# liangheming/simple_pose

Hardware: AMD Instinct MI355X
Metric: images/sec fwd+decode, ResNet50-DConv 256x192 bs=128 (higher is better)
Workload: dtype f32; 1 GPU; ResNet50-DConv 256x192 bs=128 per GPU, fp32 forward (NCHW in -> heat maps) + GaussTaylor decode, eval-mode BN, conditioned random weights; images_per_gpu=128, global_batch=128, parallelism=replicas x1 (no collective), ranks=1 process(es), one per GPU, launch=stream launches, tile_table=profiles/r06_dconv_f32_tiles.json, batches_in_flight=2, decode=in line, HSA_ENABLE_IPC_MODE_LEGACY=0

## Files before the change

### include/simple_pose_hip.h

```cpp
#ifndef SIMPLE_POSE_HIP_H
#define SIMPLE_POSE_HIP_H

#include <stdint.h>

#ifdef __cplusplus
extern "C" {
#endif

#define SP_OK 0
#define SP_EINVAL (-1)
#define SP_ELAUNCH (-2)

#define SP_ABI_VERSION 36

#define SP_CONV_RELU 0x1u
#define SP_CONV_OUT_NCHW 0x2u
#define SP_CONV_PIXEL_SHUFFLE 0x4u
#define SP_CONV_OUT_F32 0x10u
#define SP_CONV_BN_Y_MASK 0x20u
#define SP_CONV_BF16 0x8u
#define SP_CONV_HARDSWISH 0x40u
#define SP_CONV_OUT_SLICE 0x80u

typedef struct sp_conv_desc {
// ... 26 lines not shown


int sp_nchw_to_nhwc4(const float* x_nchw, float* y_nhwc4, int batch, int channels, int h, int w, void* stream);

int sp_conv2d_fwd(const sp_conv_desc* desc, const void* x, const void* w_packed, const float* scale,
                  const float* shift, const void* residual, void* y, void* stream);

int sp_conv_set_tap_skip(int on);

int sp_conv3x3_direct_ok(const sp_conv_desc* desc);
int sp_conv3x3_direct(const sp_conv_desc* desc, const void* x, const void* w_packed, const float* scale, const float* shift,
                      const void* residual, void* y, void* stream);

int sp_basic_block_c32_ok(const sp_conv_desc* desc);
int sp_basic_block_c32(const sp_conv_desc* desc, const void* x, const void* w1_packed, const float* scale1, const float* shift1,
                       const void* w2_packed, const float* scale2, const float* shift2, void* y, void* stream);

int sp_basic_block_c64_ok(const sp_conv_desc* desc);
int sp_basic_block_c64(const sp_conv_desc* desc, const void* x, const void* w1_packed, const float* scale1, const float* shift1,
                       const void* w2_packed, const float* scale2, const float* shift2, void* y, void* stream);

int sp_dual_pw_bf16_ok(int64_t rows, int c_main, int c_short, int c_out);
int sp_dual_pw_f32_ok(int64_t rows, int c_main, int c_short, int c_out);
int sp_dual_pw_f32(const float* a_main, const float* w_main_packed, const float* scale_main, const float* shift_main, const float* a_short,
                   const float* w_short_packed, const float* scale_short, const float* shift_short, float* y, int64_t rows, int c_main, int c_short,
                   int c_out, int relu, void* stream);
int sp_dual_pw_bf16(const void* a_main, const void* w_main_packed, const float* scale_main, const float* shift_main, const void* a_short,
                    const void* w_short_packed, const float* scale_short, const float* shift_short, void* y, int64_t rows, int c_main, int c_short,
                    int c_out, int relu, void* stream);
int sp_pw_chain_f32_ok(int64_t rows, int c_mid, int c_out, int c_next);
int sp_pw_chain_f32(const float* t, const float* w3_packed, const float* scale3, const float* shift3, const float* residual, float* y,
                    const float* w1_packed, const float* scale1, const float* shift1, float* t_next, int64_t rows, int c_mid, int c_out, int c_next,
                    void* stream);
int sp_bottleneck_c64_ok(const sp_conv_desc* desc);
int sp_bottleneck_c64(const sp_conv_desc* desc, const void* x, const void* w1_packed, const float* scale1, const float* shift1,
                      const void* w2_packed, const float* scale2, const float* shift2, const void* w3_packed, const float* scale3,
                      const float* shift3, void* y, void* stream);

int sp_stem7_pool_ok(int batch, int h, int w);
int sp_stem7_pool(const float* x, const void* w_packed, int k_pad, const float* scale, const float* shift, void* y, int bf16,
                  int batch, int h, int w, void* stream);
int sp_stem7_pool_u8(const unsigned char* crops_bgr, const float* mean_rgb_host, const void* w_packed, int k_pad, const float* scale,
                     const float* shift, void* y, int bf16, int batch, int h, int w, void* stream);

int sp_hrnet_transition1_ok(int c_in, int h, int w);
int sp_hrnet_transition1(const void* x, int batch, int h, int w, const void* wa_packed, int k_pad, const float* scale_a, const float* shift_a,
                         const void* wb_packed, const float* scale_b, const float* shift_b, void* y_hi, void* y_lo, void* stream);
int sp_hrnet_stem_ok(int batch, int h, int w);
int sp_hrnet_stem(const float* x, const void* w1_packed, int k1_pad, const float* scale1, const float* shift1, const void* w2_packed,
                  const float* scale2, const float* shift2, void* y, int batch, int h, int w, void* stream);

int sp_conv2d_pw_ok(const sp_conv_desc* desc);

int sp_conv2d_ring_ok(const sp_conv_desc* desc);

int sp_conv2d_kernel_name(const sp_conv_desc* desc, int has_residual, int variant, char* buf, int cap);

int sp_conv2d_default_tile(const sp_conv_desc* desc, int* tile_m, int* tile_n);

int sp_maxpool3x3s2_nhwc(const float* x, float* y, int batch, int h, int w, int c, void* stream);

int sp_pixel_shuffle2_nhwc(const float* x, float* y, int batch, int h, int w, int c, void* stream);

int sp_global_avg_pool_nhwc(const float* x, float* y, int batch, int hw, int c, void* stream);
int sp_se_gate_add_relu_nhwc(const float* x, const float* gate_logits, const float* identity, float* y, int batch, int hw,
                             int c, void* stream);
// ... 360 lines not shown
```

### simple_pose_amd/_lib.py

```python
from __future__ import annotations

import ctypes
import os
from ctypes import c_double, c_float, c_int, c_int32, c_int64, c_uint32, c_void_p

from .build import LIB_PATH as _DEFAULT_LIB_PATH

LIB_PATH = os.environ.get("SIMPLE_POSE_HIP_LIB", _DEFAULT_LIB_PATH)

SP_CONV_RELU = 0x1
SP_CONV_OUT_NCHW = 0x2
SP_CONV_PIXEL_SHUFFLE = 0x4
SP_CONV_BF16 = 0x8
SP_CONV_OUT_F32 = 0x10
SP_CONV_BN_Y_MASK = 0x20
SP_CONV_HARDSWISH = 0x40
SP_CONV_OUT_SLICE = 0x80
SP_LETTERBOX_FOCUS, SP_LETTERBOX_U8 = 0, 1
SP_YOLO_NMS_MAX_CANDIDATES, SP_YOLO_NMS_MAX_DET = 32768, 1024
SP_COCO_MAX_JOINTS, SP_COCO_MAX_GT_PER_IMAGE, SP_COCO_MAX_DT_PER_IMAGE, SP_COCO_MAX_DETS = 64, 128, 2048, 32
SP_COCO_DT_XY_F64, SP_COCO_DT_SCORE_F64, SP_COCO_GT_CROWD, SP_COCO_GT_IGNORE = 1, 2, 1, 2
CONV_TILES =((128, 128), (64, 128), (128, 64), (64, 64), (256, 64), (128, 32))
ABI_VERSION = 36
SP_CONV_KERNEL_IGEMM, SP_CONV_KERNEL_RING, SP_CONV_KERNEL_PW, SP_CONV_KERNEL_RING_LW, SP_CONV_KERNEL_RING_LW4 = 0, 1, 2, 3, 4
# ... 138 lines not shown
    "sp_pixel_unshuffle2_nhwc_bf16": (c_int, [_P, _P, c_int, c_int, c_int, c_int, _P]),
    "sp_maxpool3x3s2_idx_nhwc": (c_int, [_P, c_int, _P, _P, c_int, c_int, c_int, c_int, _P]),
    "sp_maxpool3x3s2_bwd_idx_nhwc": (c_int, [_P, _P, c_int, _P, c_int, c_int, c_int, c_int, _P]),
    "sp_nchw_to_nhwc_pad": (c_int, [_P, _P, c_int, c_int, c_int, c_int, c_int, c_int, _P]),
    "sp_warp_affine_u8c3": (c_int, [_P, c_int, c_int, _P, c_int, _P, c_int, c_int, _P]),
    "sp_warp_affine_batch_u8c3_to_nchw_f32": (c_int, [_P, _P, _P, _P, c_int, c_int, c_int, ctypes.POINTER(c_float), _P, _P, _P]),
    "sp_conv2d_bn_stats_rows": (c_int, [ctypes.POINTER(ConvDesc), ctypes.POINTER(c_int)]),
    "sp_conv2d_fwd_bn_stats": (c_int, [ctypes.POINTER(ConvDesc), _P, _P, _P, _P, _P, c_int, _P]),
    "sp_conv2d_fwd_bn_stats_abn": (c_int, [ctypes.POINTER(ConvDesc), _P, _P, _P, _P, _P, _P, _P, _P, _P, _P, _P, c_int, _P]),
    "sp_bn_train_stats_from_conv": (c_int, [_P, _P, c_int, c_int, c_int64, c_int, c_float, c_float, _P, _P, _P, _P, _P]),
    "sp_conv2d_dgrad_bn_bwd_stats": (c_int, [ctypes.POINTER(ConvDesc), _P, _P, _P, _P, _P, _P, _P, _P, _P, _P, c_int, _P]),
    "sp_conv2d_dgrad_bn_bwd_stats2": (c_int, [ctypes.POINTER(ConvDesc), _P, _P, _P, _P, _P, _P, _P, _P, _P, _P, _P, _P, _P, _P, c_int, _P]),
    "sp_conv2d_dgrad_bn_bwd_stats_macc": (c_int, [ctypes.POINTER(ConvDesc), _P, _P, _P, _P, _P, _P, _P, _P, _P, _P, _P, _P, _P, _P, _P, c_int, _P]),
    "sp_conv2d_dgrad_phases": (c_int, [ctypes.POINTER(ConvDesc), c_int, _P, ctypes.POINTER(_P), _P, _P, _P, _P, _P, _P, _P, _P, _P, _P, _P, _P, c_int, _P]),
    "sp_bn_sums_from_conv": (c_int, [_P, _P, c_int, c_int, c_int, _P, _P]),
    "sp_bn_fold_apply_nhwc": (c_int, [_P, c_int, _P, _P, c_int, c_int, c_int64, c_float, c_float, _P, _P, _P, _P, c_int64, c_int, c_int, _P, _P, _P, _P, _P, _P]),
    "sp_bn_fold_bwd_apply_nhwc": (c_int, [_P, c_int, _P, _P, _P, _P, _P, c_int, c_int, _P, _P, _P, c_int64, c_int64, c_int, _P, _P, _P, _P, _P, _P, c_int, _P]),
    "sp_bn_bwd_sums_from_conv": (c_int, [_P, _P, c_int, c_int, c_int, _P, _P, _P]),
    "sp_bn_bwd_sums_from_conv_pair": (c_int, [_P, _P, _P, c_int, c_int, c_int, _P, _P, _P, _P, _P]),
    "sp_u8hwc_bgr_to_nhwc": (c_int, [_P, _P, c_int, c_int, c_int, c_int, _P, _P]),
    "sp_nchw_to_nhwc4_bf16": (c_int, [_P, _P, c_int, c_int, c_int, c_int, _P]),
    "sp_conv3x3_direct_ok": (c_int, [ctypes.POINTER(ConvDesc)]),
    "sp_conv3x3_direct": (c_int, [ctypes.POINTER(ConvDesc), _P, _P, _P, _P, _P, _P, _P]),
    "sp_basic_block_c32_ok": (c_int, [ctypes.POINTER(ConvDesc)]),
    "sp_basic_block_c32": (c_int, [ctypes.POINTER(ConvDesc), _P, _P, _P, _P, _P, _P, _P, _P, _P]),
    "sp_basic_block_c64_ok": (c_int, [ctypes.POINTER(ConvDesc)]),
    "sp_basic_block_c64": (c_int, [ctypes.POINTER(ConvDesc), _P, _P, _P, _P, _P, _P, _P, _P, _P]),
    "sp_dual_pw_bf16_ok": (c_int, [c_int64, c_int, c_int, c_int]),
    "sp_dual_pw_f32_ok": (c_int, [c_int64, c_int, c_int, c_int]),
    "sp_dual_pw_f32": (c_int, [_P, _P, _P, _P, _P, _P, _P, _P, _P, c_int64, c_int, c_int, c_int, c_int, _P]),
    "sp_dual_pw_bf16": (c_int, [_P, _P, _P, _P, _P, _P, _P, _P, _P, c_int64, c_int, c_int, c_int, c_int, _P]),
    "sp_pw_chain_f32_ok": (c_int, [c_int64, c_int, c_int, c_int]),
    "sp_pw_chain_f32": (c_int, [_P, _P, _P, _P, _P, _P, _P, _P, _P, _P, c_int64, c_int, c_int, c_int, _P]),
    "sp_bottleneck_c64_ok": (c_int, [ctypes.POINTER(ConvDesc)]),
    "sp_conv2d_pw_ok": (c_int, [ctypes.POINTER(ConvDesc)]),
    "sp_hrnet_stem_ok": (c_int, [c_int, c_int, c_int]),
    "sp_hrnet_stem": (c_int, [_P, _P, c_int, _P, _P, _P, _P, _P, _P, c_int, c_int, c_int, _P]),
    "sp_hrnet_transition1_ok": (c_int, [c_int, c_int, c_int]),
    "sp_hrnet_transition1": (c_int, [_P, c_int, c_int, c_int, _P, c_int, _P, _P, _P, _P, _P, _P, _P, _P]),
    "sp_stem7_pool_ok": (c_int, [c_int, c_int, c_int]),
    "sp_stem7_pool": (c_int, [_P, _P, c_int, _P, _P, _P, c_int, c_int, c_int, c_int, _P]),
    "sp_stem7_pool_u8": (c_int, [_P, ctypes.POINTER(ctypes.c_float), _P, c_int, _P, _P, _P, c_int, c_int, c_int, c_int, _P]),
    "sp_bottleneck_c64": (c_int, [ctypes.POINTER(ConvDesc), _P, _P, _P, _P, _P, _P, _P, _P, _P, _P, _P, _P]),
    "sp_masked_mse": (c_int, [_P, _P, _P, c_int, c_int, c_int, _P, _P, _P, _P]),
    "sp_conv_packed_dims": (c_int, [c_int, c_int, c_int, ctypes.POINTER(c_int), ctypes.POINTER(c_int)]),
    "sp_pack_conv_weights": (c_int, [_P, c_int, c_int, c_int, c_int, c_int, c_int, c_int, c_int, c_int, c_int, _P, c_int, _P]),
    "sp_pack_conv_weights_grouped": (c_int, [_P, c_int, c_int, c_int, c_int, c_int, _P, c_int, _P]),
    "sp_pack_conv_weights_grouped_taps": (c_int, [_P, c_int, c_int, c_int, c_int, c_int, c_int, c_int, c_int, c_int, c_int, c_int, c_int, _P, c_int, _P]),
    "sp_conv2d_wgrad_grouped_workspace": (c_int, [c_int, c_int, c_int, c_int, c_int, c_int, ctypes.POINTER(c_int64)]),
    "sp_conv2d_wgrad_grouped": (c_int, [_P, _P, c_int, c_int, c_int, c_int, c_int, c_int, c_int, c_int, c_int, c_int, c_int, c_int, _P, _P, c_int64, _P]),
    "sp_pack_deconv_k4s2p1": (c_int, [_P, c_int, c_int, c_int, _P, c_int, _P]),
    "sp_fold_bn": (c_int, [_P, _P, _P, _P, c_int, c_float, c_int, _P, _P, _P]),
    "sp_yolo_letterbox": (c_int, [_P, c_int, c_int, c_int, c_int, c_int, c_int, c_int, c_int, c_int, c_int, _P, _P]),
    "sp_yolo_focus_nchw": (c_int, [_P, c_int, c_int, c_int, _P, _P]),
    "sp_yolo_spp_nhwc": (c_int, [_P, c_int, c_int, c_int, c_int, c_int, _P]),
    "sp_upsample2_slice_nhwc": (c_int, [_P, c_int, _P, c_int, c_int, c_int, c_int, c_int, _P]),
    "sp_yolo_head_decode": (c_int, [_P, _P, _P, c_int, ctypes.POINTER(c_int32), c_int, c_int, c_int, ctypes.POINTER(c_float), ctypes.POINTER(c_float), _P, _P]),
    "sp_yolo_nms_workspace": (c_int, [c_int, ctypes.POINTER(c_int64)]),
    "sp_yolo_nms": (c_int, [_P, c_int, c_int, c_int, c_float, c_float, c_int, c_int, c_int, c_int, _P, c_int64, _P, ctypes.POINTER(c_int32), ctypes.POINTER(c_int32), _P]),
    "sp_yolo_boxes_to_source": (c_int, [_P, c_int, c_float, c_float, c_float, c_float, c_float, _P]),
    "sp_yolo_nms_device": (c_int, [_P, c_int, c_int, c_int, c_float, c_float, c_int, c_int, c_int, c_int, _P, c_int64, _P, _P, _P, _P]),
    "sp_topdown_plan": (c_int, [_P, _P, c_int, c_int, c_int, c_float, c_int, c_int, c_int, c_int, c_int, _P, _P, _P, _P, _P, _P, _P, _P, _P, _P, _P]),
    "sp_warp_affine_plan_u8c3": (c_int, [_P, c_int, c_int, c_int, _P, _P, _P, c_int, _P, c_int, c_int, _P]),
    "sp_mirror_w": (c_int, [_P, _P, c_int64, c_int, c_int, _P]),
    "sp_heat_map_flip_merge": (c_int, [_P, _P, ctypes.POINTER(c_int32), c_int, c_int, c_int, c_int, c_int, _P, _P]),
    "sp_track_associate": (c_int, [_P, _P, _P, _P, _P, _P, c_int, c_int, ctypes.POINTER(c_double), c_double, c_int, c_int, _P, _P, _P, _P, _P, _P, _P, _P,
# ... 104 lines not shown
```

### simple_pose_amd/csrc/conv_pw.hip

```cpp
#include "sp_common.h"

namespace {

struct PwArgs {
    const float* x;
    const float* w;
    const float* scale;
    const float* shift;
    const float* res;
    float* y;
    int M, N, nchunks, tiles_m, relu;
    unsigned x_bytes, y_bytes;
};

constexpr int BM = 64;
constexpr int TRS = 68;
constexpr unsigned OOB = 0x80000000u;

template <int K>
__global__ __launch_bounds__(256, 1) void conv_pw_kernel(const PwArgs p) {
    constexpr int CH = K / 4;
    constexpr int NG = K / 8;
    constexpr int APT = BM * CH / 256;
    extern __shared__ __align__(16) float smem[];
// ... 403 lines not shown
#pragma unroll
        for (int i = 0; i < RT; ++i) fy[0][i] = yfrag(i, 0);
#pragma unroll
        for (int g = 0; g < NG1; ++g) {
            if (g + 1 < NG1) {
#pragma unroll
                for (int i = 0; i < RT; ++i) fy[(g + 1) & 1][i] = yfrag(i, g + 1);
            }
#pragma unroll
            for (int s = 0; s < 4; ++s)
#pragma unroll
                for (int i = 0; i < RT; ++i) c[i] = __builtin_amdgcn_mfma_f32_32x32x2f32(fy[g & 1][i][s], fw[g][s], c[i], 0, 0, 0);
        }
#pragma unroll
        for (int i = 0; i < RT; ++i)
#pragma unroll
            for (int r = 0; r < 16; ++r) {
                float v = c[i][r] * s1v + h1v;
                v = v > 0.f ? v : 0.f;
                t2[(i * 32 + (r & 3) + 8 * (r >> 2) + 4 * fh) * T2S + fr] = v;
            }
#pragma unroll
        for (int it = 0; it < RT * 4; ++it) {
            const int lr = it * 8 + (lane >> 3), cc = (lane & 7) * 4;
            const int row = m0 + ri0 * 32 + lr;
            const unsigned o = row < p.M ? (unsigned)(((size_t)row * NEXT + cn * 32 + cc) * 4) : OOB;
            const f32x4 v = *reinterpret_cast<const f32x4*>(t2 + lr * T2S + cc);
            __builtin_amdgcn_raw_buffer_store_b128(__builtin_bit_cast(u32x4, v), tnr, o, 0, 0);
        }
        __syncthreads();
    }
}

template <int NEXT>
int launch_pw_chain(const PwChainArgs& a, hipStream_t stream) {
    constexpr int lds = (2 * BM * 64 + 4 * BM * TRS + 4 * (NEXT / 64) * 32 * T2S) * 4;
    if (sp_reserve_lds<&conv_pw_chain_kernel<64, NEXT>>(lds, "conv_pw_chain")) return SP_ELAUNCH;
    int slots = sp_device_cus();
    if (slots < 1) slots = 1;
    if (slots > a.tiles_m) slots = a.tiles_m;
    const int rounds = (a.tiles_m + slots - 1) / slots;
    slots = (a.tiles_m + rounds - 1) / rounds;
    hipLaunchKernelGGL((conv_pw_chain_kernel<64, NEXT>), dim3(slots), dim3(256), lds, stream, a);
    return sp_check_launch("conv_pw_chain_kernel");
}

template <int K>
int launch_pw_dual(const PwDualArgs& a, hipStream_t stream) {
    constexpr int lds = (4 * BM * K + 4 * BM * TRS) * 4;
    if (sp_reserve_lds<&conv_pw_dual_kernel<K>>(lds, "conv_pw_dual")) return SP_ELAUNCH;
    int slots = sp_device_cus() / a.nchunks;
    if (slots < 1) slots = 1;
    if (slots > a.tiles_m) slots = a.tiles_m;
    const int rounds = (a.tiles_m + slots - 1) / slots;
    slots = (a.tiles_m + rounds - 1) / rounds;
    hipLaunchKernelGGL(conv_pw_dual_kernel<K>, dim3(slots * a.nchunks), dim3(256), lds, stream, a);
    return sp_check_launch("conv_pw_dual_kernel");
}

template <int K>
int launch_pw(const PwArgs& a, hipStream_t stream) {
    constexpr int lds = (2 * BM * K + 4 * BM * TRS) * 4;
    if (sp_reserve_lds<&conv_pw_kernel<K>>(lds, "conv_pw")) return SP_ELAUNCH;
    int slots = sp_device_cus() / a.nchunks;
    if (slots < 1) slots = 1;
    if (slots > a.tiles_m) slots = a.tiles_m;
// ... 46 lines not shown
    SP_REQUIRE(a_main && w_main_packed && a_short && w_short_packed && y, "sp_dual_pw_f32: null pointer");
    SP_REQUIRE(sp_dual_pw_f32_ok(rows, c_main, c_short, c_out), "sp_dual_pw_f32: two fp32 1x1 stride-1 products of 64 channels each into a multiple of 256 (got %d + %d -> %d, %lld rows)",
               c_main, c_short, c_out, (long long)rows);
    SP_REQUIRE(y != a_main && y != a_short, "sp_dual_pw_f32: y must not alias an input");
    if (sp_name_query_active()) { sp_name_query_set("conv_pw_dual_kernel<64>"); return SP_OK; }
    PwDualArgs a;
    a.x_main = a_main; a.x_short = a_short; a.w_main = w_main_packed; a.w_short = w_short_packed;
    a.s_main = scale_main; a.h_main = shift_main; a.s_short = scale_short; a.h_short = shift_short; a.y = y;
    a.M = (int)rows; a.N = c_out; a.nchunks = c_out / 256; a.tiles_m = (int)((rows + BM - 1) / BM); a.relu = relu ? 1 : 0;
    a.x_bytes = (unsigned)(rows * 64 * 4); a.y_bytes = (unsigned)(rows * c_out * 4);
    return launch_pw_dual<64>(a, (hipStream_t)stream);
}

extern "C" int sp_pw_chain_f32_ok(int64_t rows, int c_mid, int c_out, int c_next) {
    return rows > 0 && rows * (int64_t)c_out <= (1ll << 29) && c_mid == 64 && c_out == 256 && (c_next == 64 || c_next == 128);
}

extern "C" int sp_pw_chain_f32(const float* t, const float* w3_packed, const float* scale3, const float* shift3, const float* residual, float* y,
                               const float* w1_packed, const float* scale1, const float* shift1, float* t_next, int64_t rows, int c_mid, int c_out,
                               int c_next, void* stream) {
    SP_REQUIRE(t && w3_packed && residual && y && w1_packed && t_next, "sp_pw_chain_f32: null pointer");
    SP_REQUIRE(sp_pw_chain_f32_ok(rows, c_mid, c_out, c_next),
               "sp_pw_chain_f32: an fp32 1x1 product 64 -> 256 chained into a 1x1 product 256 -> 64 or 128 (got %d -> %d -> %d, %lld rows)", c_mid, c_out,
               c_next, (long long)rows);
    SP_REQUIRE(y != t && y != residual && t_next != t && t_next != residual && t_next != y, "sp_pw_chain_f32: y and t_next must not alias an input or each other");
    if (sp_name_query_active()) { sp_name_query_set("conv_pw_chain_kernel<64, %d>", c_next); return SP_OK; }
    PwChainArgs a;
    a.x = t; a.w = w3_packed; a.scale = scale3; a.shift = shift3; a.res = residual; a.y = y;
    a.w1 = w1_packed; a.scale1 = scale1; a.shift1 = shift1; a.t = t_next;
    a.M = (int)rows; a.tiles_m = (int)((rows + BM - 1) / BM);
    a.x_bytes = (unsigned)(rows * 64 * 4); a.y_bytes = (unsigned)(rows * 256 * 4); a.t_bytes = (unsigned)(rows * c_next * 4);
    return c_next == 64 ? launch_pw_chain<64>(a, (hipStream_t)stream) : launch_pw_chain<128>(a, (hipStream_t)stream);
}
```

### simple_pose_amd/engine.py

```python
from __future__ import annotations

import ctypes
import os

from dataclasses import dataclass, field
from typing import Dict, List, Optional, Tuple

import torch

from . import _lib, conv_geometry
from ._lib import ConvDesc, SP_CONV_BF16, SP_CONV_HARDSWISH, SP_CONV_OUT_NCHW, SP_CONV_OUT_SLICE, SP_CONV_PIXEL_SHUFFLE, SP_CONV_RELU
from .conv_geometry import n_pad_for, round_up as _round_up

BN_EPS = 1e-5


class HipPacker:

    @staticmethod
    def _dims(c_out: int, k: int, bf16: bool) -> Tuple[int, int]:
        n_pad, k_pad = ctypes.c_int(0), ctypes.c_int(0)
        _lib.check(_lib.lib().sp_conv_packed_dims(c_out, k, int(bf16), ctypes.byref(n_pad), ctypes.byref(k_pad)), "sp_conv_packed_dims")
        return n_pad.value, k_pad.value

# ... 147 lines not shown
                last_writer[dn] = i
            for n in op.reads() + op.writes():
                touched.setdefault(store(n), []).append(i)
        records = sorted({j for w in waits for j in w})
        tails: Dict[int, int] = {}
        for i, op in enumerate(self.ops):
            tails[op.lane] = i
        self._sync[key] = (waits, set(records), tails)
        return self._sync[key]

    def _lane_streams(self, key, n_lanes: int, device=None) -> list:
        pool = self._streams.setdefault(str(key), [])
        while len(pool) < n_lanes - 1:
            pool.append(torch.cuda.Stream(device=device if device is not None else key))
        return pool

    def _launch(self, lib, op: Op, bufs, B: int, stream) -> None:
        P = _lib.ptr
        if op.kind == "conv":
            op.desc.batch = B
            fn = lib.sp_conv3x3_direct if op.direct else lib.sp_conv2d_fwd
            _lib.check(fn(op.desc, P(bufs[op.src]), P(op.w), P(op.scale), P(op.shift),
                          P(bufs[op.res]) if op.res else None, P(bufs[op.dst]) + 4 * op.c0, stream), op.name)
        elif op.kind in ("bb32", "bb64"):
            op.desc.batch = B
            w2, scale2, shift2 = op.args
            _lib.check((lib.sp_basic_block_c32 if op.kind == "bb32" else lib.sp_basic_block_c64)(op.desc, P(bufs[op.src]), P(op.w), P(op.scale), P(op.shift), P(w2), P(scale2), P(shift2),
                                              P(bufs[op.dst]), stream), op.name)
        elif op.kind == "bneck64":
            op.desc.batch = B
            w1, s1, h1, w3, s3, h3 = op.args
            _lib.check(lib.sp_bottleneck_c64(op.desc, P(bufs[op.src]), P(w1), P(s1), P(h1), P(op.w), P(op.scale), P(op.shift), P(w3), P(s3), P(h3),
                                             P(bufs[op.dst]), stream), op.name)
        elif op.kind == "dual1x1":
            w_s, s_s, h_s, rows_per_image, relu = op.args
            fn = lib.sp_dual_pw_bf16 if op.w.element_size() == 2 else lib.sp_dual_pw_f32
            _lib.check(fn(P(bufs[op.src]), P(op.w), P(op.scale), P(op.shift), P(bufs[op.res]), P(w_s), P(s_s), P(h_s), P(bufs[op.dst]),
                                           B * rows_per_image, 64, 64, 256, relu, stream), op.name)
        elif op.kind == "pwchain":
            w1, s1, h1, rows_per_image, c_next, _ = op.args
            _lib.check(lib.sp_pw_chain_f32(P(bufs[op.src]), P(op.w), P(op.scale), P(op.shift), P(bufs[op.res]), P(bufs[op.dst]), P(w1), P(s1), P(h1),
                                           P(bufs[op.dst2]), B * rows_per_image, 64, 256, c_next, stream), op.name)
        elif op.kind == "stem7":
            h, w, k_pad, unfused = op.args
            src = bufs[op.src]
            if src.dtype == torch.uint8:
                mean = (ctypes.c_float * 3)(0.485, 0.456, 0.406)
                _lib.check(lib.sp_stem7_pool_u8(P(src), mean, P(op.w), k_pad, P(op.scale), P(op.shift), P(bufs[op.dst]), int(self.dtype == "bf16"),
                                                B, h, w, stream), op.name)
            else:
                _lib.check(lib.sp_stem7_pool(P(src), P(op.w), k_pad, P(op.scale), P(op.shift), P(bufs[op.dst]), int(self.dtype == "bf16"),
                                             B, h, w, stream), op.name)
        elif op.kind == "htrans":
            h, w, k_pad, wb, sb, hb, _ = op.args
            _lib.check(lib.sp_hrnet_transition1(P(bufs[op.src]), B, h, w, P(op.w), k_pad, P(op.scale), P(op.shift), P(wb), P(sb), P(hb),
                                                P(bufs[op.dst]), P(bufs[op.dst2]), stream), op.name)
        elif op.kind == "hstem":
            h, w, k1_pad, w2, s2, h2, unfused = op.args
            src = bufs[op.src]
            if src.dtype == torch.uint8:
                tmp = dict(bufs)
                for u in unfused[:-1]:
                    uh, uw, uc = self.shapes[u.dst]
                    tmp[u.dst] = torch.empty(B * uh * uw * uc, dtype=torch.bfloat16, device=src.device)
                for u in unfused:
                    self._launch(lib, u, tmp, B, stream)
            else:
                _lib.check(lib.sp_hrnet_stem(P(src), P(op.w), k1_pad, P(op.scale), P(op.shift), P(w2), P(s2), P(h2), P(bufs[op.dst]), B, h, w,
                                             stream), op.name)
        elif op.kind == "maxpool":
            h, w, c = op.args
            fn = lib.sp_maxpool3x3s2_nhwc_bf16 if self.dtype == "bf16" else lib.sp_maxpool3x3s2_nhwc
# ... 427 lines not shown
                out = self.decoder(out, trans_inv)
            if self._done[k] is None:
                self._done[k] = torch.cuda.Event()
            self._done[k].record(st)
        return out

    def sync(self) -> None:
        for ev in self._done:
            if ev is not None:
                torch.cuda.current_stream().wait_event(ev)

    def close(self) -> None:
        torch.cuda.synchronize()
        mine = range(self._slot0, self._slot0 + self.depth)
        for key in [k for k in self.prog._pools if len(k) == 3 and k[2] in mine]:
            del self.prog._pools[key]
        for table in (self.prog._streams, self.prog._events):
            for key in [k for k in table if "/" in k and k.rsplit("/", 1)[1].isdigit() and int(k.rsplit("/", 1)[1]) in mine]:
                del table[key]
        self._hm = [None] * self.depth


class ProgramBuilder:

    def __init__(self, in_h: int, in_w: int, dtype: str = "fp32", packer=None):
        if dtype not in ("fp32", "bf16"):
            raise ValueError(dtype)
        self.packer = packer or HipPacker()
        self.fuse_blocks = False
        self.fuse_blocks64 = False
        self.fuse_bottlenecks = False
        self.fuse_tail = os.environ.get("SP_FUSE_TAIL", "1") != "0"
        self.fuse_chain = os.environ.get("SP_FUSE_CHAIN", "1") != "0"
        self.fuse_stem = True
        self.fuse_terms = True
        self.fuse_transition = True
        self.p = Program(dtype=dtype)
        self.bf16 = dtype == "bf16"
        self.cpad = 8 if self.bf16 else 4
        self.p.shapes["input"] = (in_h, in_w, 3)
        self._n = 0
        self.lane = 0

    def _add(self, op: Op) -> None:
        op.lane = self.lane
        self.p.ops.append(op)

    def _fresh(self, stem: str) -> str:
        self._n += 1
        return f"{stem}#{self._n}"

    def to_nhwc4(self, src: str) -> str:
        h, w, c = self.p.shapes[src]
        dst = self._fresh("x4")
        self.p.shapes[dst] = (h, w, 4)
        self._add(Op("to_nhwc4", src, dst, args=(c, h, w), name="to_nhwc4"))
        return dst

    def stem_pool(self, src: str, weight: torch.Tensor, scale, shift, name: str = "conv1") -> str:
        first = len(self.p.ops)
        x4 = self.to_nhwc4(src)
        y = self.conv(x4, weight, stride=2, pad=3, scale=scale, shift=shift, relu=True, name=name)
        out = self.maxpool(y)
        h, w, _ = self.p.shapes[src]
        if not (self.fuse_stem and tuple(weight.shape) == (64, 3, 7, 7) and _lib.lib().sp_stem7_pool_ok(1, h, w)):
            return out
# ... 225 lines not shown
    if (p + ".se.fc.0.weight") in sd:
        z = b.conv(t, sd[p + ".conv3.weight"], scale=s3, shift=h3, name=p + ".conv3")
        g = b.gap(z)
        g = b.conv(g, sd[p + ".se.fc.0.weight"], shift=b.packer.bias(sd[p + ".se.fc.0.bias"]), relu=True, name=p + ".se.fc.0")
        g = b.conv(g, sd[p + ".se.fc.2.weight"], shift=b.packer.bias(sd[p + ".se.fc.2.bias"]), name=p + ".se.fc.2")
        return b.se_gate(z, g, idn)
    return b.conv(t, sd[p + ".conv3.weight"], scale=s3, shift=h3, relu=True, res=idn, name=p + ".conv3")


def _res_basic_block(b: ProgramBuilder, sd, x: str, p: str, stride: int) -> str:
    s1, h1 = _bn(b, sd, p + ".bn1")
    t = b.conv(x, sd[p + ".conv1.weight"], stride=stride, pad=1, scale=s1, shift=h1, relu=True, name=p + ".conv1")
    idn = x
    if (p + ".downsample.0.weight") in sd:
        sdn, hdn = _bn(b, sd, p + ".downsample.1")
        idn = b.conv(x, sd[p + ".downsample.0.weight"], stride=stride, scale=sdn, shift=hdn, name=p + ".downsample")
    s2, h2 = _bn(b, sd, p + ".bn2")
    if (p + ".se.fc.0.weight") in sd:
        z = b.conv(t, sd[p + ".conv2.weight"], pad=1, scale=s2, shift=h2, name=p + ".conv2")
        g = b.gap(z)
        g = b.conv(g, sd[p + ".se.fc.0.weight"], shift=b.packer.bias(sd[p + ".se.fc.0.bias"]), relu=True, name=p + ".se.fc.0")
        g = b.conv(g, sd[p + ".se.fc.2.weight"], shift=b.packer.bias(sd[p + ".se.fc.2.bias"]), name=p + ".se.fc.2")
        return b.se_gate(z, g, idn)
    return b.conv(t, sd[p + ".conv2.weight"], pad=1, scale=s2, shift=h2, relu=True, res=idn, name=p + ".conv2")


def _plain_pointwise(d) -> bool:
    return (d.c_in_group == 0 and d.taps_h == 1 and d.taps_w == 1 and d.stride == 1 and d.stride_x in (0, 1) and d.phases_y == 1 and d.phases_x == 1 and
            d.dy0 == 0 and d.dx0 == 0 and (d.grid_h, d.grid_w) == (d.in_h, d.in_w) == (d.out_h, d.out_w) and d.oy_mul == 1 and d.ox_mul == 1 and
            d.oy_add == 0 and d.ox_add == 0 and d.k_pad == d.c_in and d.n_pad == d.c_out and d.out_c == d.c_out)


def _fuse_pw_chains(b: "ProgramBuilder", sd) -> None:
    if b.bf16 or not b.fuse_chain:
        return
    ops, out, i = b.p.ops, [], 0
    while i < len(ops):
        a, c = ops[i], ops[i + 1] if i + 1 < len(ops) else None
        ok = (c is not None and a.kind == "conv" and c.kind == "conv" and a.lane == c.lane and a.name.endswith(".conv3") and c.name.endswith(".conv1") and
              a.res is not None and c.res is None and c.src == a.dst and not a.direct and not c.direct and a.c0 == 0 and c.c0 == 0 and
              a.scale is not None and a.shift is not None and c.scale is not None and c.shift is not None)
        if ok:
            blk, da, dc = a.name[:-len(".conv3")], a.desc, c.desc
            ok = ((blk + ".downsample.0.weight") not in sd and (blk + ".se.fc.0.weight") not in sd and _plain_pointwise(da) and _plain_pointwise(dc) and
                  da.flags == SP_CONV_RELU and dc.flags == SP_CONV_RELU and da.c_in == 64 and da.c_out == 256 and dc.c_in == 256 and
                  dc.c_out in (64, 128) and tuple(a.w.shape) == (256, 64) and tuple(c.w.shape) == (dc.c_out, 256) and
                  _lib.lib().sp_pw_chain_f32_ok(da.grid_h * da.grid_w, 64, 256, dc.c_out))
        if ok:
            out.append(Op("pwchain", a.src, a.dst, res=a.res, dst2=c.dst, w=a.w, scale=a.scale, shift=a.shift,
                          args=(c.w, c.scale, c.shift, da.grid_h * da.grid_w, dc.c_out, (a, c)), name=a.name + "+" + c.name, flops=a.flops + c.flops,
                          lane=a.lane))
            i += 2
        else:
            out.append(a)
            i += 1
    b.p.ops[:] = out


def resnet_program(sd: Dict[str, torch.Tensor], head: str, in_h: int = 256, in_w: int = 192,
                   blocks=(3, 4, 6, 3), dtype: str = "fp32", packer=None, fuse_bottlenecks: bool = False, fuse_stem: bool = True,
                   fuse_chain: bool = False) -> Program:
    b = ProgramBuilder(in_h, in_w, dtype, packer)
    b.fuse_bottlenecks = fuse_bottlenecks
    b.fuse_tail = fuse_bottlenecks and b.fuse_tail
    b.fuse_stem = fuse_stem
    s, h = _bn(b, sd, "bn1")
    x = b.stem_pool("input", sd["conv1.weight"], s, h, name="conv1")
    basic = "layer1.0.conv3.weight" not in sd
    for li, n in enumerate(blocks, start=1):
        for bi in range(n):
            x = (_res_basic_block if basic else _bottleneck)(b, sd, x, f"layer{li}.{bi}", 2 if (bi == 0 and li > 1) else 1)
    if fuse_chain and not basic:
        _fuse_pw_chains(b, sd)
    J = sd["final_layer.weight"].shape[0]
    if head == "dconv":
        for idx in (0, 3, 6):
            s, h = _bn(b, sd, f"deconv_layers.{idx + 1}")
            x = b.deconv_k4s2p1(x, sd[f"deconv_layers.{idx}.weight"], scale=s, shift=h, relu=True,
                                name=f"deconv_layers.{idx}")
        b.conv(x, sd["final_layer.weight"], shift=b.packer.bias(sd["final_layer.bias"]), out_nchw=True,
               dst="heat", name="final_layer")
    elif head == "duc":
        x = b.pixel_shuffle(x)
        for idx in (1, 2):
            s, h = _bn(b, sd, f"duc_layers.{idx}.bn", pixel_shuffle=True)
            x = b.conv(x, sd[f"duc_layers.{idx}.conv.weight"], pad=1, scale=s, shift=h, relu=True, pixel_shuffle=True,
                       name=f"duc_layers.{idx}")
        b.conv(x, sd["final_layer.weight"], pad=1, shift=b.packer.bias(sd["final_layer.bias"]), out_nchw=True,
               dst="heat", name="final_layer")
    else:
        raise ValueError(head)
    hh, ww, _ = b.p.shapes["heat"]
    b.p.out_shape = (J, hh, ww)
    return b.p


def _basic_block(b: ProgramBuilder, sd, x: str, p: str) -> str:
    s1, h1 = _bn(b, sd, p + ".bn1")
    s2, h2 = _bn(b, sd, p + ".bn2")
    fused = b.basic_block_c32(x, sd[p + ".conv1.weight"], s1, h1, sd[p + ".conv2.weight"], s2, h2, name=p)
    if fused is not None:
        return fused
    t = b.conv(x, sd[p + ".conv1.weight"], pad=1, scale=s1, shift=h1, relu=True, name=p + ".conv1")
    return b.conv(t, sd[p + ".conv2.weight"], pad=1, scale=s2, shift=h2, relu=True, res=x, name=p + ".conv2")

# ... 247 lines not shown
```

### simple_pose_amd/nets/_resnet_base.py

```python
from __future__ import annotations

from typing import Optional

import torch
from torch import nn

from .. import engine
from .._lib import HipLibraryError, require_cuda_f32
from ..metrics.flip import COCO_JOINT_PAIRS, merge_flipped, mirror_input, pairs_to_perm


class _Bottleneck(nn.Module):
    expansion = 4

    def __init__(self, inplanes: int, planes: int, stride: int, with_downsample: bool, with_se: bool = False, width: int = 0, groups: int = 1):
        super().__init__()
        width = width or planes
        self.conv1 = nn.Conv2d(inplanes, width, 1, bias=False)
        self.bn1 = nn.BatchNorm2d(width)
        self.conv2 = nn.Conv2d(width, width, 3, stride=stride, padding=1, groups=groups, bias=False)
        self.bn2 = nn.BatchNorm2d(width)
        self.conv3 = nn.Conv2d(width, planes * 4, 1, bias=False)
        self.bn3 = nn.BatchNorm2d(planes * 4)
        if with_downsample:
# ... 51 lines not shown
        Block = _Bottleneck if block == "bottleneck" else _BasicBlock
        for li, (planes, n) in enumerate(zip((64, 128, 256, 512), self.BLOCKS), start=1):
            blocks = []
            for bi in range(n):
                stride = 2 if (bi == 0 and li > 1) else 1
                down = bi == 0 and (stride != 1 or inplanes != planes * Block.expansion)
                blocks.append(Block(inplanes, planes, stride, with_downsample=down, with_se=(reduction and down),
                                    width=planes * width_per_group // 64 * groups, groups=groups))
                inplanes = planes * Block.expansion
            setattr(self, f"layer{li}", nn.Sequential(*blocks))
        self._build_head(inplanes, num_classes)
        self._init_like_reference()
        self.compute_dtype = "fp32"
        self.autotune = True
        self._program: Optional[engine.Program] = None
        self._program_key = None

    def _init_like_reference(self):
        for m in self.modules():
            if isinstance(m, (nn.Conv2d, nn.ConvTranspose2d)):
                nn.init.normal_(m.weight, std=0.001)
                if m.bias is not None:
                    nn.init.constant_(m.bias, 0)
            elif isinstance(m, nn.BatchNorm2d):
                nn.init.constant_(m.weight, 1)
                nn.init.constant_(m.bias, 0)

    def _build_head(self, inplanes: int, num_classes: int):
        raise NotImplementedError

    fuse_bottlenecks = True
    fuse_stem = True
    fuse_chain = True

    def _tensors_key(self, x):
        sd = self.state_dict(keep_vars=True)
        return (tuple(x.shape[2:]), str(x.device), self.compute_dtype, self.fuse_bottlenecks, self.fuse_stem, self.fuse_chain) + tuple((v.data_ptr(), v._version) for v in sd.values())

    def hip_program(self, x: torch.Tensor) -> engine.Program:
        key = self._tensors_key(x)
        if self._program is None or key != self._program_key:
            sd = {k: v.detach() for k, v in self.state_dict(keep_vars=True).items()}
            for k, v in sd.items():
                if v.device != x.device:
                    raise HipLibraryError(f"parameter {k} is on {v.device} but the input is on {x.device}; call .to(device)")
            self._program = engine.resnet_program(sd, self.HEAD, in_h=x.shape[2], in_w=x.shape[3], blocks=self.BLOCKS,
                                                   dtype=self.compute_dtype, fuse_bottlenecks=self.fuse_bottlenecks, fuse_stem=self.fuse_stem,
                                                   fuse_chain=self.fuse_chain)
            self._program_key = key
        return self._program

    def forward(self, x: torch.Tensor) -> torch.Tensor:
        x = require_cuda_f32(x, "input")
        if x.dim() != 4 or x.shape[1] != 3 or x.shape[2] % 32 or x.shape[3] % 32:
            raise ValueError(f"expected [B,3,H,W] with H,W multiples of 32, got {tuple(x.shape)}")
        if self.training:
            return self._forward_train(x)
        prog = self.hip_program(x)
        if self.autotune and x.shape[0] >= 16 and x.shape[0] >= 4 * prog.tuned_for_batch:
            prog.autotune(x)
        return prog.run(x)

    def _forward_train(self, x: torch.Tensor) -> torch.Tensor:
        return train_forward(self, x)

    def forward_crops(self, crops: torch.Tensor, flip_test: bool = False, joint_pairs=COCO_JOINT_PAIRS, shift_heatmap: bool = False) -> torch.Tensor:
        return forward_uint8_crops(self, crops, flip_test, joint_pairs, shift_heatmap)


def train_forward(self, x: torch.Tensor) -> torch.Tensor:
    from ..train import PoseTrainer
    import torch.distributed as dist
    if dist.is_available() and dist.is_initialized() and dist.get_world_size() > 1 and not getattr(self, "_warned_local_bn", False):
        import warnings
        warnings.warn("simple_pose_amd: model(x) in train() mode under an initialised process group uses per-rank BatchNorm statistics "
                      "(sync_bn: False behaviour); PoseTrainer(model, process_group=..., sync_bn=True).step() is the SyncBatchNorm path")
        self._warned_local_bn = True
    key = (x.shape[2], x.shape[3], str(x.device), self.compute_dtype)
    tr = getattr(self, "_trainer", None)
    if tr is None or self._trainer_key != key or not tr.still_owns_parameters():
        tr = PoseTrainer(self, in_h=x.shape[2], in_w=x.shape[3], dtype="bf16" if self.compute_dtype == "bf16" else "fp32",
# ... 55 lines not shown
```

Measured before the change: 11880 images/s.

## Fuse stage-opening bottleneck dual 1x1 tail with next block's conv1

Adds a HIP kernel that computes the two 1x1 products of a 64-channel stage-opening bottleneck (conv3 plus downsample shortcut), adds them with ReLU, writes the 256-channel output, and chains it straight into the next block's 256->64 conv1 from LDS. The engine pass also extends chaining to conv3 ops of downsample blocks as 'tailchain'. The aim is to avoid re-reading the 256-channel activation from global memory and to save a kernel launch at the stage boundaries. In exchange the new kernel keeps many weights in registers at one workgroup per CU, which can lower occupancy, and it only covers one shape.

Result: no change. 11940 images/s, median of 6 (+0.5%).

```diff
diff --git a/include/simple_pose_hip.h b/include/simple_pose_hip.h
--- a/include/simple_pose_hip.h
+++ b/include/simple_pose_hip.h
@@ -82,6 +82,11 @@
 int sp_pw_chain_f32(const float* t, const float* w3_packed, const float* scale3, const float* shift3, const float* residual, float* y,
                     const float* w1_packed, const float* scale1, const float* shift1, float* t_next, int64_t rows, int c_mid, int c_out, int c_next,
                     void* stream);
+int sp_dual_pw_chain_f32_ok(int64_t rows, int c_main, int c_short, int c_out, int c_next);
+int sp_dual_pw_chain_f32(const float* a_main, const float* w_main_packed, const float* scale_main, const float* shift_main, const float* a_short,
+                         const float* w_short_packed, const float* scale_short, const float* shift_short, float* y, const float* w1_packed,
+                         const float* scale1, const float* shift1, float* t_next, int64_t rows, int c_main, int c_short, int c_out, int c_next,
+                         void* stream);
 int sp_bottleneck_c64_ok(const sp_conv_desc* desc);
 int sp_bottleneck_c64(const sp_conv_desc* desc, const void* x, const void* w1_packed, const float* scale1, const float* shift1,
                       const void* w2_packed, const float* scale2, const float* shift2, const void* w3_packed, const float* scale3,
diff --git a/simple_pose_amd/_lib.py b/simple_pose_amd/_lib.py
--- a/simple_pose_amd/_lib.py
+++ b/simple_pose_amd/_lib.py
@@ -194,6 +194,8 @@
     "sp_dual_pw_bf16": (c_int, [_P, _P, _P, _P, _P, _P, _P, _P, _P, c_int64, c_int, c_int, c_int, c_int, _P]),
     "sp_pw_chain_f32_ok": (c_int, [c_int64, c_int, c_int, c_int]),
     "sp_pw_chain_f32": (c_int, [_P, _P, _P, _P, _P, _P, _P, _P, _P, _P, c_int64, c_int, c_int, c_int, _P]),
+    "sp_dual_pw_chain_f32_ok": (c_int, [c_int64, c_int, c_int, c_int, c_int]),
+    "sp_dual_pw_chain_f32": (c_int, [_P] * 13 + [c_int64, c_int, c_int, c_int, c_int, _P]),
     "sp_bottleneck_c64_ok": (c_int, [ctypes.POINTER(ConvDesc)]),
     "sp_conv2d_pw_ok": (c_int, [ctypes.POINTER(ConvDesc)]),
     "sp_hrnet_stem_ok": (c_int, [c_int, c_int, c_int]),
diff --git a/simple_pose_amd/csrc/conv_pw.hip b/simple_pose_amd/csrc/conv_pw.hip
--- a/simple_pose_amd/csrc/conv_pw.hip
+++ b/simple_pose_amd/csrc/conv_pw.hip
@@ -459,6 +459,189 @@
     }
 }
 
+struct PwDualChainArgs {
+    const float* x_main;
+    const float* x_short;
+    const float* w_main;
+    const float* w_short;
+    const float *s_main, *h_main, *s_short, *h_short;
+    float* y;
+    const float* w1;
+    const float* scale1;
+    const float* shift1;
+    float* t;
+    int M, tiles_m;
+    unsigned x_bytes, y_bytes, t_bytes;
+};
+
+template <int K, int NEXT>
+__global__ __launch_bounds__(256, 1) void conv_pw_dual_chain_kernel(const PwDualChainArgs p) {
+    static_assert(K == 64 && NEXT == 64, "the dual tail of a 64-channel stage-opening Bottleneck into a 64-channel conv1");
+    constexpr int N = 256;
+    constexpr int CH = K / 4;
+    constexpr int NG = K / 8;
+    constexpr int NG1 = N / 8;
+    constexpr int APT = BM * CH / 256;
+    extern __shared__ __align__(16) float smem[];
+    float* const As = smem;
+    const int tid = threadIdx.x, lane = tid & 63, wave = tid >> 6;
+    float* const ys = smem + 4 * BM * K;
+    float* const tr = ys + wave * (BM * TRS);
+    float* const t2 = ys + 4 * BM * TRS + wave * (32 * T2S);
+    const int fr = lane & 31, fh = lane >> 5;
+    const int slot = blockIdx.x, nslots = gridDim.x;
+    const int nbase = wave * 64;
+    const int cn = wave >> 1, ri0 = wave & 1;
+
+    const __amdgpu_buffer_rsrc_t xr0 = __builtin_amdgcn_make_buffer_rsrc(const_cast<float*>(p.x_main), (short)0, p.x_bytes, 0x00020000);
+    const __amdgpu_buffer_rsrc_t xr1 = __builtin_amdgcn_make_buffer_rsrc(const_cast<float*>(p.x_short), (short)0, p.x_bytes, 0x00020000);
+    const __amdgpu_buffer_rsrc_t yr = __builtin_amdgcn_make_buffer_rsrc(p.y, (short)0, p.y_bytes, 0x00020000);
+    const __amdgpu_buffer_rsrc_t tnr = __builtin_amdgcn_make_buffer_rsrc(p.t, (short)0, p.t_bytes, 0x00020000);
+
+    float fb[2][NG][2][4];
+#pragma unroll
+    for (int q = 0; q < 2; ++q)
+#pragma unroll
+        for (int g = 0; g < NG; ++g)
+#pragma unroll
+            for (int n = 0; n < 2; ++n) {
+                const f32x4 t = *reinterpret_cast<const f32x4*>((q ? p.w_short : p.w_main) + (size_t)(nbase + n * 32 + fr) * K + 8 * g + 4 * fh);
+                fb[q][g][n][0] = t[0]; fb[q][g][n][1] = t[1]; fb[q][g][n][2] = t[2]; fb[q][g][n][3] = t[3];
+            }
+    float fw[NG1][4];
+#pragma unroll
+    for (int g = 0; g < NG1; ++g) {
+        const f32x4 t = *reinterpret_cast<const f32x4*>(p.w1 + (size_t)(cn * 32 + fr) * N + 8 * g + 4 * fh);
+        fw[g][0] = t[0]; fw[g][1] = t[1]; fw[g][2] = t[2]; fw[g][3] = t[3];
+    }
+    float s3v[2], h3v[2], sdv[2], hdv[2];
+#pragma unroll
+    for (int n = 0; n < 2; ++n) {
+        const int ch = nbase + n * 32 + fr;
+        s3v[n] = p.s_main ? p.s_main[ch] : 1.f;  h3v[n] = p.h_main ? p.h_main[ch] : 0.f;
+        sdv[n] = p.s_short ? p.s_short[ch] : 1.f; hdv[n] = p.h_short ? p.h_short[ch] : 0.f;
+    }
+    const float s1v = p.scale1 ? p.scale1[cn * 32 + fr] : 1.f, h1v = p.shift1 ? p.shift1[cn * 32 + fr] : 0.f;
+    const int c4 = (lane & 15) * 4, rsub = lane >> 4;
+
+    auto swz = [](int row, int chunk) { return row * K + ((chunk ^ (row & (CH - 1))) << 2); };
+    u32x4 sa[2][APT];
+    auto load_a = [&](int mt) {
+        const unsigned base = (unsigned)mt * (BM * K * 4);
+#pragma unroll
+        for (int i = 0; i < APT; ++i) {
+            sa[0][i] = __builtin_amdgcn_raw_buffer_load_b128(xr0, base + (unsigned)((tid + 256 * i) * 16), 0, 0);
+            sa[1][i] = __builtin_amdgcn_raw_buffer_load_b128(xr1, base + (unsigned)((tid + 256 * i) * 16), 0, 0);
+        }
+    };
+    auto park_a = [&](int buf) {
+#pragma unroll
+        for (int q = 0; q < 2; ++q)
+#pragma unroll
+            for (int i = 0; i < APT; ++i) {
+                const int e = tid + 256 * i;
+                *reinterpret_cast<u32x4*>(As + (buf * 2 + q) * (BM * K) + swz(e / CH, e % CH)) = sa[q][i];
+            }
+    };
+
+    int mt = slot;
+    if (mt >= p.tiles_m) return;
+    load_a(mt);
+    park_a(0);
+    __syncthreads();
+    int cur = 0;
+    for (; mt < p.tiles_m; mt += nslots, cur ^= 1) {
+        const int m0 = mt * BM;
+        const bool more = mt + nslots < p.tiles_m;
+        if (more) load_a(mt + nslots);
+#pragma unroll
+        for (int i = 0; i < 2; ++i) {
+            f32x16 acc[2][2];
+#pragma unroll
+            for (int q = 0; q < 2; ++q)
+#pragma unroll
+                for (int n = 0; n < 2; ++n)
+#pragma unroll
+                    for (int r = 0; r < 16; ++r) acc[q][n][r] = 0.f;
+#pragma unroll
+            for (int q = 0; q < 2; ++q) {
+                const float* a = As + (cur * 2 + q) * (BM * K);
+                f32x4 fa[2];
+                fa[0] = *reinterpret_cast<const f32x4*>(a + swz(i * 32 + fr, fh));
+#pragma unroll
+                for (int g = 0; g < NG; ++g) {
+                    if (g + 1 < NG) fa[(g + 1) & 1] = *reinterpret_cast<const f32x4*>(a + swz(i * 32 + fr, 2 * (g + 1) + fh));
+#pragma unroll
+                    for (int s = 0; s < 4; ++s)
+#pragma unroll
+                        for (int n = 0; n < 2; ++n)
+                            acc[q][n] = __builtin_amdgcn_mfma_f32_32x32x2f32(fa[g & 1][s], fb[q][g][n][s], acc[q][n], 0, 0, 0);
+                }
+            }
+#pragma unroll
+            for (int n = 0; n < 2; ++n)
+#pragma unroll
+                for (int r = 0; r < 16; ++r) {
+                    const float vd = acc[1][n][r] * sdv[n] + hdv[n];
+                    float v = acc[0][n][r] * s3v[n] + h3v[n];
+                    v += vd;
+                    v = v > 0.f ? v : 0.f;
+                    tr[(i * 32 + (r & 3) + 8 * (r >> 2) + 4 * fh) * TRS + n * 32 + fr] = v;
+                }
+#pragma unroll
+            for (int it = 8 * i; it < 8 * i + 8; ++it) {
+                const int row = m0 + it * 4 + rsub;
+                const unsigned off = row < p.M ? (unsigned)(((size_t)row * N + nbase + c4) * 4) : OOB;
+                const f32x4 v = *reinterpret_cast<const f32x4*>(tr + (it * 4 + rsub) * TRS + c4);
+                __builtin_amdgcn_raw_buffer_store_b128(__builtin_bit_cast(u32x4, v), yr, off, 0, 0);
+            }
+        }
+        if (more) park_a(cur ^ 1);
+        __syncthreads();
+
+        f32x16 c;
+#pragma unroll
+        for (int r = 0; r < 16; ++r) c[r] = 0.f;
+        auto yfrag = [&](int g) { return *reinterpret_cast<const f32x4*>(ys + (g >> 3) * (BM * TRS) + (ri0 * 32 + fr) * TRS + 8 * (g & 7) + 4 * fh); };
+        f32x4 fy[2];
+        fy[0] = yfrag(0);
+#pragma unroll
+        for (int g = 0; g < NG1; ++g) {
+            if (g + 1 < NG1) fy[(g + 1) & 1] = yfrag(g + 1);
+#pragma unroll
+            for (int s = 0; s < 4; ++s) c = __builtin_amdgcn_mfma_f32_32x32x2f32(fy[g & 1][s], fw[g][s], c, 0, 0, 0);
+        }
+#pragma unroll
+        for (int r = 0; r < 16; ++r) {
+            float v = c[r] * s1v + h1v;
+            v = v > 0.f ? v : 0.f;
+            t2[((r & 3) + 8 * (r >> 2) + 4 * fh) * T2S + fr] = v;
+        }
+#pragma unroll
+        for (int it = 0; it < 4; ++it) {
+            const int lr = it * 8 + (lane >> 3), cc = (lane & 7) * 4;
+            const int row = m0 + ri0 * 32 + lr;
+            const unsigned o = row < p.M ? (unsigned)(((size_t)row * NEXT + cn * 32 + cc) * 4) : OOB;
+            const f32x4 v = *reinterpret_cast<const f32x4*>(t2 + lr * T2S + cc);
+            __builtin_amdgcn_raw_buffer_store_b128(__builtin_bit_cast(u32x4, v), tnr, o, 0, 0);
+        }
+        __syncthreads();
+    }
+}
+
+int launch_pw_dual_chain(const PwDualChainArgs& a, hipStream_t stream) {
+    constexpr int lds = (4 * BM * 64 + 4 * BM * TRS + 4 * 32 * T2S) * 4;
+    static_assert(lds <= 160 * 1024, "one workgroup's LDS");
+    if (sp_reserve_lds<&conv_pw_dual_chain_kernel<64, 64>>(lds, "conv_pw_dual_chain")) return SP_ELAUNCH;
+    int slots = sp_device_cus();
+    if (slots < 1) slots = 1;
+    if (slots > a.tiles_m) slots = a.tiles_m;
+    const int rounds = (a.tiles_m + slots - 1) / slots;
+    slots = (a.tiles_m + rounds - 1) / rounds;
+    hipLaunchKernelGGL((conv_pw_dual_chain_kernel<64, 64>), dim3(slots), dim3(256), lds, stream, a);
+    return sp_check_launch("conv_pw_dual_chain_kernel");
+}
+
 template <int NEXT>
 int launch_pw_chain(const PwChainArgs& a, hipStream_t stream) {
     constexpr int lds = (2 * BM * 64 + 4 * BM * TRS + 4 * (NEXT / 64) * 32 * T2S) * 4;
@@ -571,3 +754,27 @@
     a.x_bytes = (unsigned)(rows * 64 * 4); a.y_bytes = (unsigned)(rows * 256 * 4); a.t_bytes = (unsigned)(rows * c_next * 4);
     return c_next == 64 ? launch_pw_chain<64>(a, (hipStream_t)stream) : launch_pw_chain<128>(a, (hipStream_t)stream);
 }
+
+extern "C" int sp_dual_pw_chain_f32_ok(int64_t rows, int c_main, int c_short, int c_out, int c_next) {
+    return rows > 0 && rows * (int64_t)c_out <= (1ll << 29) && c_main == 64 && c_short == 64 && c_out == 256 && c_next == 64;
+}
+
+extern "C" int sp_dual_pw_chain_f32(const float* a_main, const float* w_main_packed, const float* scale_main, const float* shift_main, const float* a_short,
+                                    const float* w_short_packed, const float* scale_short, const float* shift_short, float* y, const float* w1_packed,
+                                    const float* scale1, const float* shift1, float* t_next, int64_t rows, int c_main, int c_short, int c_out, int c_next,
+                                    void* stream) {
+    SP_REQUIRE(a_main && w_main_packed && a_short && w_short_packed && y && w1_packed && t_next, "sp_dual_pw_chain_f32: null pointer");
+    SP_REQUIRE(sp_dual_pw_chain_f32_ok(rows, c_main, c_short, c_out, c_next),
+               "sp_dual_pw_chain_f32: two fp32 1x1 products of 64 channels each into 256, chained into a 1x1 product 256 -> 64 (got %d + %d -> %d -> %d, %lld rows)",
+               c_main, c_short, c_out, c_next, (long long)rows);
+    SP_REQUIRE(y != a_main && y != a_short && t_next != a_main && t_next != a_short && t_next != y,
+               "sp_dual_pw_chain_f32: y and t_next must not alias an input or each other");
+    if (sp_name_query_active()) { sp_name_query_set("conv_pw_dual_chain_kernel<64, %d>", c_next); return SP_OK; }
+    PwDualChainArgs a;
+    a.x_main = a_main; a.x_short = a_short; a.w_main = w_main_packed; a.w_short = w_short_packed;
+    a.s_main = scale_main; a.h_main = shift_main; a.s_short = scale_short; a.h_short = shift_short; a.y = y;
+    a.w1 = w1_packed; a.scale1 = scale1; a.shift1 = shift1; a.t = t_next;
+    a.M = (int)rows; a.tiles_m = (int)((rows + BM - 1) / BM);
+    a.x_bytes = (unsigned)(rows * 64 * 4); a.y_bytes = (unsigned)(rows * 256 * 4); a.t_bytes = (unsigned)(rows * c_next * 4);
+    return launch_pw_dual_chain(a, (hipStream_t)stream);
+}
diff --git a/simple_pose_amd/engine.py b/simple_pose_amd/engine.py
--- a/simple_pose_amd/engine.py
+++ b/simple_pose_amd/engine.py
@@ -203,12 +203,16 @@
             w1, s1, h1, w3, s3, h3 = op.args
             _lib.check(lib.sp_bottleneck_c64(op.desc, P(bufs[op.src]), P(w1), P(s1), P(h1), P(op.w), P(op.scale), P(op.shift), P(w3), P(s3), P(h3),
                                              P(bufs[op.dst]), stream), op.name)
-        elif op.kind == "dual1x1":
+        elif op.kind == "dual1x1" and op.dst2 is None:
             w_s, s_s, h_s, rows_per_image, relu = op.args
             fn = lib.sp_dual_pw_bf16 if op.w.element_size() == 2 else lib.sp_dual_pw_f32
             _lib.check(fn(P(bufs[op.src]), P(op.w), P(op.scale), P(op.shift), P(bufs[op.res]), P(w_s), P(s_s), P(h_s), P(bufs[op.dst]),
                                            B * rows_per_image, 64, 64, 256, relu, stream), op.name)
-        elif op.kind == "pwchain":
+        elif op.kind == "dual1x1":
+            w_s, s_s, h_s, rows_per_image, _, w1, s1, h1, c_next, _ = op.args
+            _lib.check(lib.sp_dual_pw_chain_f32(P(bufs[op.src]), P(op.w), P(op.scale), P(op.shift), P(bufs[op.res]), P(w_s), P(s_s), P(h_s), P(bufs[op.dst]),
+                                                P(w1), P(s1), P(h1), P(bufs[op.dst2]), B * rows_per_image, 64, 64, 256, c_next, stream), op.name)
+        elif op.kind in ("pwchain", "tailchain"):
             w1, s1, h1, rows_per_image, c_next, _ = op.args
             _lib.check(lib.sp_pw_chain_f32(P(bufs[op.src]), P(op.w), P(op.scale), P(op.shift), P(bufs[op.res]), P(bufs[op.dst]), P(w1), P(s1), P(h1),
                                            P(bufs[op.dst2]), B * rows_per_image, 64, 256, c_next, stream), op.name)
@@ -702,6 +706,7 @@
         self.fuse_bottlenecks = False
         self.fuse_tail = os.environ.get("SP_FUSE_TAIL", "1") != "0"
         self.fuse_chain = os.environ.get("SP_FUSE_CHAIN", "1") != "0"
+        self.fuse_chain_tail = self.fuse_chain
         self.fuse_stem = True
         self.fuse_terms = True
         self.fuse_transition = True
@@ -993,35 +998,51 @@
 
 
 def _fuse_pw_chains(b: "ProgramBuilder", sd) -> None:
-    if b.bf16 or not b.fuse_chain:
+    if b.bf16 or not (b.fuse_chain or b.fuse_chain_tail):
         return
     ops, out, i = b.p.ops, [], 0
     while i < len(ops):
         a, c = ops[i], ops[i + 1] if i + 1 < len(ops) else None
-        ok = (c is not None and a.kind == "conv" and c.kind == "conv" and a.lane == c.lane and a.name.endswith(".conv3") and c.name.endswith(".conv1") and
-              a.res is not None and c.res is None and c.src == a.dst and not a.direct and not c.direct and a.c0 == 0 and c.c0 == 0 and
+        kind = None
+        ok = (c is not None and a.kind in ("conv", "dual1x1") and c.kind == "conv" and a.lane == c.lane and c.name.endswith(".conv1") and a.res is not None and
+              c.res is None and c.src == a.dst and a.dst2 is None and not a.direct and not c.direct and a.c0 == 0 and c.c0 == 0 and
               a.scale is not None and a.shift is not None and c.scale is not None and c.shift is not None)
         if ok:
-            blk, da, dc = a.name[:-len(".conv3")], a.desc, c.desc
-            ok = ((blk + ".downsample.0.weight") not in sd and (blk + ".se.fc.0.weight") not in sd and _plain_pointwise(da) and _plain_pointwise(dc) and
-                  da.flags == SP_CONV_RELU and dc.flags == SP_CONV_RELU and da.c_in == 64 and da.c_out == 256 and dc.c_in == 256 and
-                  dc.c_out in (64, 128) and tuple(a.w.shape) == (256, 64) and tuple(c.w.shape) == (dc.c_out, 256) and
-                  _lib.lib().sp_pw_chain_f32_ok(da.grid_h * da.grid_w, 64, 256, dc.c_out))
-        if ok:
-            out.append(Op("pwchain", a.src, a.dst, res=a.res, dst2=c.dst, w=a.w, scale=a.scale, shift=a.shift,
-                          args=(c.w, c.scale, c.shift, da.grid_h * da.grid_w, dc.c_out, (a, c)), name=a.name + "+" + c.name, flops=a.flops + c.flops,
-                          lane=a.lane))
-            i += 2
-        else:
-            out.append(a)
-            i += 1
+            dc = c.desc
+            ok = _plain_pointwise(dc) and dc.flags == SP_CONV_RELU and dc.c_in == 256 and tuple(c.w.shape) == (dc.c_out, 256)
+        if ok and a.kind == "conv":
+            blk, da = a.name[:-len(".conv3")], a.desc
+            ok = (a.name.endswith(".conv3") and (blk + ".se.fc.0.weight") not in sd and _plain_pointwise(da) and da.flags == SP_CONV_RELU and da.c_in == 64 and
+                  da.c_out == 256 and dc.c_out in (64, 128) and tuple(a.w.shape) == (256, 64) and
+                  (da.grid_h, da.grid_w) == (dc.grid_h, dc.grid_w) and _lib.lib().sp_pw_chain_f32_ok(da.grid_h * da.grid_w, 64, 256, dc.c_out))
+            kind = "tailchain" if (blk + ".downsample.0.weight") in sd else "pwchain"
+            if ok and (b.fuse_chain_tail if kind == "tailchain" else b.fuse_chain):
+                out.append(Op(kind, a.src, a.dst, res=a.res, dst2=c.dst, w=a.w, scale=a.scale, shift=a.shift,
+                              args=(c.w, c.scale, c.shift, da.grid_h * da.grid_w, dc.c_out, (a, c)), name=a.name + "+" + c.name, flops=a.flops + c.flops,
+                              lane=a.lane))
+                i += 2
+                continue
+        elif ok:
+            w_s, s_s, h_s, rows_per_image, relu = a.args
+            ok = (b.fuse_chain_tail and a.w.element_size() == 4 and relu == 1 and rows_per_image == dc.grid_h * dc.grid_w and s_s is not None and
+                  h_s is not None and _lib.lib().sp_dual_pw_chain_f32_ok(rows_per_image, 64, 64, 256, dc.c_out))
+            if ok:
+                out.append(Op("dual1x1", a.src, a.dst, res=a.res, dst2=c.dst, w=a.w, scale=a.scale, shift=a.shift,
+                              args=(w_s, s_s, h_s, rows_per_image, relu, c.w, c.scale, c.shift, dc.c_out, (a, c)), name=a.name + "+" + c.name,
+                              flops=a.flops + c.flops, lane=a.lane))
+                i += 2
+                continue
+        out.append(a)
+        i += 1
     b.p.ops[:] = out
 
 
 def resnet_program(sd: Dict[str, torch.Tensor], head: str, in_h: int = 256, in_w: int = 192,
                    blocks=(3, 4, 6, 3), dtype: str = "fp32", packer=None, fuse_bottlenecks: bool = False, fuse_stem: bool = True,
-                   fuse_chain: bool = False) -> Program:
+                   fuse_chain: bool = False, fuse_chain_tail: Optional[bool] = None) -> Program:
     b = ProgramBuilder(in_h, in_w, dtype, packer)
+    fuse_chain_tail = fuse_chain if fuse_chain_tail is None else fuse_chain_tail
+    b.fuse_chain, b.fuse_chain_tail = b.fuse_chain and fuse_chain, b.fuse_chain_tail and fuse_chain_tail
     b.fuse_bottlenecks = fuse_bottlenecks
     b.fuse_tail = fuse_bottlenecks and b.fuse_tail
     b.fuse_stem = fuse_stem
@@ -1031,7 +1052,7 @@
     for li, n in enumerate(blocks, start=1):
         for bi in range(n):
             x = (_res_basic_block if basic else _bottleneck)(b, sd, x, f"layer{li}.{bi}", 2 if (bi == 0 and li > 1) else 1)
-    if fuse_chain and not basic:
+    if not basic:
         _fuse_pw_chains(b, sd)
     J = sd["final_layer.weight"].shape[0]
     if head == "dconv":
diff --git a/simple_pose_amd/nets/_resnet_base.py b/simple_pose_amd/nets/_resnet_base.py
--- a/simple_pose_amd/nets/_resnet_base.py
+++ b/simple_pose_amd/nets/_resnet_base.py
@@ -107,10 +107,11 @@
     fuse_bottlenecks = True
     fuse_stem = True
     fuse_chain = True
+    fuse_chain_tail = True
 
     def _tensors_key(self, x):
         sd = self.state_dict(keep_vars=True)
-        return (tuple(x.shape[2:]), str(x.device), self.compute_dtype, self.fuse_bottlenecks, self.fuse_stem, self.fuse_chain) + tuple((v.data_ptr(), v._version) for v in sd.values())
+        return (tuple(x.shape[2:]), str(x.device), self.compute_dtype, self.fuse_bottlenecks, self.fuse_stem, self.fuse_chain, self.fuse_chain_tail) + tuple((v.data_ptr(), v._version) for v in sd.values())
 
     def hip_program(self, x: torch.Tensor) -> engine.Program:
         key = self._tensors_key(x)
@@ -121,7 +122,7 @@
                     raise HipLibraryError(f"parameter {k} is on {v.device} but the input is on {x.device}; call .to(device)")
             self._program = engine.resnet_program(sd, self.HEAD, in_h=x.shape[2], in_w=x.shape[3], blocks=self.BLOCKS,
                                                    dtype=self.compute_dtype, fuse_bottlenecks=self.fuse_bottlenecks, fuse_stem=self.fuse_stem,
-                                                   fuse_chain=self.fuse_chain)
+                                                   fuse_chain=self.fuse_chain, fuse_chain_tail=self.fuse_chain_tail)
             self._program_key = key
         return self._program
 
```
